# mrjoshuak/go-jpeg2000

Measured on AMD Instinct MI355X. Metric: Mpixels/s encode+decode (4K sRGB, 5-3 lossless), higher is better.
Workload: dtype int32

## Files before the change

### go-jpeg2000_amd/csrc/ht.hip

```cpp
#include <cstdlib>

#include "ht_tables.h"
#include "j2k_internal.h"

namespace j2k {

__device__ __constant__ uint16_t c_vlc_tbl0[1024] = J2K_HT_VLC_TBL0_INIT;
__device__ __constant__ uint16_t c_vlc_tbl1[1024] = J2K_HT_VLC_TBL1_INIT;
__device__ uint16_t g_vlc_enc[2 * 4 * 16];

__global__ void ht_build_enc_table() {
    const int t = threadIdx.x;
    if (t >= 128) return;
    const int initial = t >> 6, context = (t >> 4) & 3, rho = t & 15;
    const uint16_t *tbl = initial ? c_vlc_tbl0 : c_vlc_tbl1;
    uint16_t r = 0x0001;
    for (uint32_t cwd = 0; cwd < 128; cwd++) {
        const uint16_t e = tbl[(context << 7) | cwd];
        if (((e >> 4) & 0xF) == rho && (e & 0xF) > 0) { r = (uint16_t)((cwd << 4) | (e & 0xF)); break; }
    }
    g_vlc_enc[t] = r;
}

__device__ uint16_t g_vlc_pair1[16384];
// ... 1207 lines not shown
    const v4i_ v = {a, b, c, d};
    if (J2K_DECODED_NT) __builtin_nontemporal_store(v, reinterpret_cast<v4i_ *>(p));
    else *reinterpret_cast<v4i_ *>(p) = v;
}

#ifdef J2K_DEC_STAMP
static __device__ long long g_dbg_unstuff_dummy;
#define g_dbg_unstuff S.dbg_t
#endif
struct HtDecShared {
#ifdef J2K_DEC_STAMP
    long long dbg_t;
#endif
    uint32_t mbuf[HT_DEC_MWORDS];
    uint32_t pair[HT_WALK_MAX_PAIRS];
    uint32_t ffpos[HT_MAX_FF];
    uint32_t nff;
};

__device__ uint32_t ht_loaded_bits(const HtDecShared &S, uint32_t nff, long segLen, uint32_t j) {
    const long k = 4 * (long)j;
    const long kk = k < segLen ? k : segLen;
    uint32_t f = 0, last_ff = 0;
    for (uint32_t i = 0; i < nff; i++) {
        if ((long)S.ffpos[i] + 2 <= kk) f++;
        if ((long)S.ffpos[i] == segLen - 1) last_ff = 1;
    }
    uint32_t b = (uint32_t)(8 * kk) - f;
    if (k > segLen) b += (last_ff ? 7u : 8u) + 7u * (uint32_t)(k - segLen - 1);
    return b;
}

template <bool STRIDED>
__device__ bool ht_extract_fast(HtDecShared &S, const uint8_t *__restrict__ data, long len, long scup, int w, int h,
                                int32_t *__restrict__ out, int lane, bool bigu, const uint32_t (&mpos2)[2], uint32_t total_bits,
                                const uint32_t (&raw0)[4], int os_) {
    const size_t os64 = STRIDED ? (size_t)os_ : (size_t)64, osw = STRIDED ? (size_t)os_ : (size_t)w;
    const int quadCols = (w + 3) / 4, P = (quadCols + 1) / 2, R = (h + 3) / 4, N = R * P;
    const long lcup = len;
    {
        const long segLen0 = lcup - scup;
        const long cap0 = (long)HT_DEC_MWORDS * 4 - 16;
        const uint32_t zw = bigu ? (uint32_t)HT_DEC_MWORDS
                                 : min((uint32_t)HT_DEC_MWORDS, (uint32_t)(((segLen0 < cap0 ? segLen0 : cap0) * 8) >> 5) + 3u);
        for (uint32_t i = lane; i < zw; i += 64) S.mbuf[i] = 0;
    }
    if (lane == 0) S.nff = 0;
    wave_sync();
    constexpr int PF = 4;
    {
        const long segLen = lcup - scup;
        const long maxbytes = (long)HT_DEC_MWORDS * 4 - 16;
        const long nb = segLen < maxbytes ? segLen : maxbytes;
        const long d = (long)((uintptr_t)data & 3);
        const uint32_t *wsrc = reinterpret_cast<const uint32_t *>(data - d);
        const long ndw = (d + nb + 3) >> 2;
        uint32_t off = 0, carry = 0;
        for (long j0 = 0; j0 < ndw; j0 += 64 * PF) {
            uint32_t raw[PF];
#pragma unroll
            for (int c = 0; c < PF; c++) {
                const long j = j0 + 64 * c + lane;
                if (j0 == 0) raw[c] = raw0[c];
                else raw[c] = wsrc[j < ndw ? j : ndw - 1];
            }
#pragma unroll
            for (int c = 0; c < PF; c++) {
// ... 137 lines not shown
#pragma unroll
            for (int half = 0; half < 2; half++) {
                const int drow = half * 4 + (lane >> 4), q = lane & 15;
                const int src = drow * 8 + (q >> 1);
                int o[4];
#pragma unroll
                for (int i = 0; i < 4; i++) {
                    const int a = __shfl(vals[i], src), b = __shfl(vals[4 + i], src);
                    o[i] = (q & 1) ? b : a;
                }
                const int rg = 8 * t + drow;
#ifdef J2K_DEC_NO_CODED_STORES
                if (o[0] == 0x7fffffff)
#endif
                if (rg < R) st_decoded(out + (size_t)(4 * rg) * os64 + 4 * q, o[0], o[1], o[2], o[3]);
            }
        } else if (it < N) {
            const int xb = pi * 8;
            int32_t *orow = out + (size_t)(4 * r) * osw + xb;
            if (xb + 8 <= w && (((uintptr_t)orow) & 15) == 0) {
                st_decoded(orow, vals[0], vals[1], vals[2], vals[3]);
                st_decoded(orow + 4, vals[4], vals[5], vals[6], vals[7]);
            } else {
#pragma unroll
                for (int i = 0; i < 8; i++)
                    if (xb + i < w) orow[i] = vals[i];
            }
        }
    }
    return true;
}

template <bool STRIDED>
__global__ __launch_bounds__(256) __attribute__((amdgpu_waves_per_eu(7, 8))) void ht_decode_kernel(const BlockJob *__restrict__ jobs, int njobs,
                                                        const uint8_t *__restrict__ stream, const uint64_t *__restrict__ offs,
                                                        const uint32_t *__restrict__ lens, int32_t *__restrict__ decoded,
                                                        const uint32_t *__restrict__ pairs, int coded_rows_only_) {
    const int coded_rows_only = STRIDED ? 1 : coded_rows_only_;
    __shared__ HtDecShared S4[4];
    HtDecShared &S = S4[threadIdx.x >> 6];
    const int jid = blockIdx.x * 4 + (threadIdx.x >> 6);
    if (jid >= njobs) return;
    const int lane = threadIdx.x & 63;
#ifdef J2K_DEC_STAMP
    const long long d0 = wall_clock64();
#endif
    const BlockJob J = jobs[jid];
    const int w = J.w, h = J.h;
    const int os_ = STRIDED ? J.stride : w;
    int32_t *out = decoded + J.out_off;
    const size_t n = (size_t)w * h;
    const uint32_t *rec = pairs + (size_t)jid * HT_WALK_REC;
    const uint32_t r0 = rec[lane], r1 = rec[64 + lane];
    const uint64_t my_off = offs[jid];
    const uint32_t my_len = lens[jid], my_scup = rec[HT_WALK_MAX_PAIRS];
    const uint32_t tag = __shfl(r0, 0);
    const bool fast = (tag != HT_PAIR_ZERO) && (tag != HT_PAIR_SERIAL);
    auto zero_fill = [&](bool skip_coded) {
        if (coded_rows_only) {
            if (skip_coded) return;
            const uint32_t uw = (uint32_t)w, nrow = (uint32_t)(h + 3) >> 2;
            for (uint32_t i = lane; i < uw * nrow; i += 64) out[(size_t)(i / uw) * 4 * (STRIDED ? (uint32_t)os_ : uw) + i % uw] = 0;
            return;
        }
        if (w == 64 && (J.out_off & 3) == 0) {
            if (skip_coded && lane < 16) return;
            int32_t *q = out + 4 * (size_t)lane;
            for (int i = 0; i < h / 4; i++) st_decoded(q + 256 * (size_t)i, 0, 0, 0, 0);
            const int rem = h & 3;
            if (lane < 16 * rem) st_decoded(q + 256 * (size_t)(h / 4), 0, 0, 0, 0);
        } else if ((w & 3) == 0 && (J.out_off & 3) == 0) {
            const uint32_t wq = (uint32_t)w >> 2, nq = (uint32_t)(n >> 2);
            const uint32_t dy = 64u / wq, dx = 64u % wq;
            uint32_t y = (uint32_t)lane / wq, x = (uint32_t)lane % wq;
            for (uint32_t i = lane; i < nq; i += 64) {
                if (!skip_coded || (y & 3)) st_decoded(out + 4 * (size_t)i, 0, 0, 0, 0);
// ... 140 lines not shown
        const uint16_t *tbl = initial ? c_vlc_tbl0 : c_vlc_tbl1;
        for (int qx = 0; qx < quadCols; qx += 2) {
            uint32_t vlcVal = rev_fetch(vlc);
            const uint32_t qinf = tbl[vlcVal & 0x7F];
            const uint32_t rho = (qinf >> 4) & 0xF, uOff1 = (qinf >> 3) & 1;
            rev_advance(vlc, qinf & 0xF);
            vlcVal = rev_fetch(vlc);
            const uint32_t qinf2 = tbl[((rho >> 2) << 7) | (vlcVal & 0x7F)];
            const uint32_t rho2 = (qinf2 >> 4) & 0xF, uOff2 = (qinf2 >> 3) & 1;
            rev_advance(vlc, qinf2 & 0xF);
            uint32_t u[2] = {1, 1};
            const uint32_t mode = (uOff1 << 1) | uOff2;
            if (mode > 0) {
                vlcVal = rev_fetch(vlc);
                rev_advance(vlc, decode_uvlc(vlcVal, mode, u, initial));
            }
            for (int q = 0; q < 2; q++) {
                const uint32_t r = q ? rho2 : rho, emb = u[q];
                const int base = (qx + q) * 4;
                for (int i = 0; i < 4 && base + i < w; i++) {
                    if (!((r >> i) & 1)) continue;
                    const uint32_t magVal = fwd_fetch(ms);
                    const uint32_t mag = (magVal & (shl32(1, emb) - 1)) + shl32(1, emb - 1);
                    fwd_advance(ms, emb);
                    const uint32_t sign = fwd_fetch(ms) & 1;
                    fwd_advance(ms, 1);
                    out[(size_t)y * (STRIDED ? (size_t)os_ : (size_t)w) + base + i] = sign ? (int32_t)(0u - mag) : (int32_t)mag;
                }
            }
        }
    }
}

static bool g_tables_ready[16] = {false};

static hipError_t ht_tables_ready(hipStream_t s) {
    int dev = 0;
    hipError_t e = hipGetDevice(&dev);
    if (e != hipSuccess) return e;
    if (dev < 0 || dev >= 16) return hipErrorInvalidDevice;
    if (g_tables_ready[dev]) return hipSuccess;
    hipLaunchKernelGGL(ht_build_enc_table, dim3(1), dim3(128), 0, s);
    hipLaunchKernelGGL(ht_build_pair_table, dim3(64), dim3(256), 0, s);
    if ((e = hipGetLastError()) != hipSuccess) return e;
    if ((e = hipFuncSetAttribute(reinterpret_cast<const void *>(ht_walk_kernel), hipFuncAttributeMaxDynamicSharedMemorySize,
                                 (int)sizeof(HtWalkShared))) != hipSuccess) return e;
    if ((e = hipStreamSynchronize(s)) != hipSuccess) return e;
    g_tables_ready[dev] = true;
    return hipSuccess;
}

hipError_t launch_ht_encode(hipStream_t s, const BlockJob *jobs, int njobs, const int32_t *coef, uint8_t *slots,
                            uint32_t *lens, uint8_t *numbps, int *fault, uint32_t *maglens, const HtUJob *utab, int nunique,
                            const int *alias_ids, int waves) {
    if (njobs <= 0) return hipSuccess;
    hipError_t e;
    if ((e = ht_tables_ready(s)) != hipSuccess) return e;
    const int n = utab ? nunique : njobs;
    if (waves == 4 && utab && alias_ids)
        hipLaunchKernelGGL(ht_encode_wg_kernel, dim3(n), dim3(256), 0, s, n, coef, slots, lens, numbps, fault, maglens, utab, alias_ids);
    else
        hipLaunchKernelGGL(ht_encode_kernel, dim3(n), dim3(64), 0, s, jobs, n, coef, slots, lens, numbps, fault, maglens, utab, alias_ids);
    return hipGetLastError();
}

hipError_t launch_ht_encode_stream(hipStream_t s, const BlockJob *jobs, int njobs, const int32_t *coef, uint8_t *stream,
                                   uint64_t *offs, uint32_t *lens, uint8_t *numbps, uint64_t *status, uint32_t epoch, int *fault) {
    if (njobs <= 0) return hipSuccess;
    hipError_t e;
    if ((e = ht_tables_ready(s)) != hipSuccess) return e;
    hipLaunchKernelGGL(ht_encode_stream_kernel, dim3(njobs), dim3(64), 0, s, jobs, njobs, coef, stream,
                       reinterpret_cast<unsigned long long *>(offs), lens, numbps, reinterpret_cast<unsigned long long *>(status), epoch, fault);
    return hipGetLastError();
}
int ht_fast_max_samples() { return HT_FAST_MAX_SAMPLES; }

size_t ht_decode_scratch_words(int njobs) { return (size_t)njobs * (HT_WALK_REC + HT_VBITS_WORDS); }

hipError_t launch_ht_decode(hipStream_t s, const BlockJob *jobs, int njobs, const uint8_t *stream, const uint64_t *offs,
                            const uint32_t *lens, int32_t *decoded, uint32_t *scratch, int coded_rows_only, const BlockJob *placed_jobs) {
    if (njobs <= 0) return hipSuccess;
    hipError_t e;
    if ((e = ht_tables_ready(s)) != hipSuccess) return e;
    uint32_t *pairs = scratch, *vbits = scratch + (size_t)njobs * HT_WALK_REC;
    for (int rep_ = 0; rep_ < dev_reps(32); rep_++)
    hipLaunchKernelGGL(ht_vlcprep_kernel, dim3((njobs + 3) / 4), dim3(256), 0, s, jobs, njobs, stream, offs, lens, vbits, pairs);
    if ((e = hipGetLastError()) != hipSuccess) return e;
    for (int rep_ = 0; rep_ < dev_reps(64); rep_++)
    hipLaunchKernelGGL(ht_walk_kernel, dim3((njobs + HT_WALK_BLOCKS - 1) / HT_WALK_BLOCKS), dim3(256), sizeof(HtWalkShared), s, jobs, njobs, vbits, pairs);
    if ((e = hipGetLastError()) != hipSuccess) return e;
    for (int rep_ = 0; rep_ < dev_reps(128); rep_++)
    if (placed_jobs) hipLaunchKernelGGL(ht_decode_kernel<true>, dim3((njobs + 3) / 4), dim3(256), 0, s, placed_jobs, njobs, stream, offs, lens, decoded, pairs, 1);
    else
    hipLaunchKernelGGL(ht_decode_kernel<false>, dim3((njobs + 3) / 4), dim3(256), 0, s, jobs, njobs, stream, offs, lens, decoded, pairs, coded_rows_only);
    return hipGetLastError();
}

}
```

### go-jpeg2000_amd/csrc/j2k_ctx.cpp

```cpp
#include "j2k_host.h"

using namespace j2k;

int fail(j2k_ctx *ctx, int status, const char *msg) {
    if (ctx) ctx->last_error = msg ? msg : "";
    return status;
}
int fail_hip(j2k_ctx *ctx, hipError_t e, const char *where) {
    char buf[256];
    snprintf(buf, sizeof(buf), "%s: %s", where, hipGetErrorString(e));
    if (ctx) ctx->last_error = buf;
    return J2K_ERR_HIP;
}

extern "C" const char *j2k_ctx_last_error(j2k_ctx *ctx) { return ctx ? ctx->last_error.c_str() : ""; }

std::atomic<int> g_mq_ctxs{0};
bool mq_throughput_mode() { return g_mq_ctxs.load(std::memory_order_relaxed) >= 2; }
struct CtxOption { const char *name; bool (*set)(j2k_ctx *, long); };
static const std::vector<CtxOption> &ctx_options() {
#define OPT(name, cond, stmt) CtxOption{name, [](j2k_ctx *c, long v) -> bool { (void)c; if (!(cond)) return false; stmt; return true; }}
    static const std::vector<CtxOption> T = {
        OPT("plane_wg3", v == 0 || v == 1, c->plane_wg3 = v != 0),
        OPT("pix_fuse", v >= 0 && v <= 2, c->pix_fuse = (int)v),
        OPT("plane_wg", v == 0 || v == 4 || v == 8, c->plane_wg = (int)v),
        OPT("l0_fuse", v == 0 || v == 8 || v == 10 || v == 16, c->l0_fuse = (int)v),
        OPT("l0_wg", v == 0 || v == 4 || v == 8, c->l0_wg = (int)v),
        OPT("plane_wg97", v == 0 || v == 8, c->plane_wg97 = (int)v),
        OPT("l0_wg97_inv", v == 0 || v == 6 || v == 8 || v == 10 || v == 12, c->l0_wg97_inv = (int)v),
        OPT("l0_wg97", v == 0 || (v >= 6 && v <= 16 && v % 2 == 0), c->l0_wg97 = (int)v),
        OPT("l0_xcd", v == 0 || v == 1, c->l0_xcd = v != 0),
        OPT("l0_deal", v == 0 || v == 1, c->l0_deal = v != 0),
        OPT("ht_alias", v == 0 || v == 1, c->ht_alias = v != 0),
        OPT("ht_enc_waves", v == 1 || v == 4, c->ht_enc_waves = (int)v),
        OPT("l0_inv_wpe", v >= 5 && v <= 7, c->l0_inv_wpe = (int)v),
        OPT("l0_wg_inv", v == 0 || v == 1, c->l0_wg_inv = v != 0),
        OPT("l0_wg_invw", v == 0 || v == 4 || v == 8, c->l0_wg_invw = (int)v),
        OPT("l0_xcd_group", v >= 0 && v <= 4096, c->l0_xcd_group = (int)v),
        OPT("l0_store", v == 0 || v == 1 || v == 2 || v == 4, c->l0_store = (int)v),
        OPT("fuse_compact", v == 0 || v == 1, c->fuse_compact = v != 0),
        OPT("deep", v == 0 || v == 1, c->use_deep = v != 0),
        OPT("deep_min_planes", v >= 0 && v <= 1000000, c->deep_min_planes = (int)v),
        OPT("deep_mid", v == 0 || v == 1, c->deep_mid = v != 0),
        OPT("deep_mid_inv", v >= 0 && v <= 2, c->deep_mid_inv = (int)v),
        OPT("mega", v >= 0 && v <= 2, c->mega = (int)v),
        OPT("t1_split", v == 0 || v == 1, c->t1_split = v != 0),
        OPT("t1_sym_mb", v >= 0, c->t1_sym_mb = v),
        OPT("t1_dec_general", v == 0 || v == 1, c->t1_dec_general = v != 0),
        OPT("t1_dec_split", v >= -1, c->t1_dec_split = (int)v),
        OPT("t1_dec_lanes", v >= 0 && v <= 2, c->t1_dec_lanes = (int)v),
        OPT("t1_lanes", v >= 0 && v <= 64, c->t1_lanes = (int)v),
        OPT("t2_parallel", v == 0 || v == 1, c->t2_parallel = v != 0),
    };
#undef OPT
    return T;
}
extern "C" int j2k_ctx_set_option(j2k_ctx *ctx, const char *name, long value) {
    if (!ctx || !name) return J2K_ERR_INVALID_ARG;
    for (const CtxOption &o : ctx_options())
        if (!strcmp(o.name, name)) return o.set(ctx, value) ? J2K_OK : fail(ctx, J2K_ERR_INVALID_ARG, "j2k_ctx_set_option: value out of range");
    return fail(ctx, J2K_ERR_INVALID_ARG, "j2k_ctx_set_option: no such option");
}

extern "C" int j2k_ctx_create(int device, j2k_ctx **out) {
    if (!out) return J2K_ERR_INVALID_ARG;
    *out = nullptr;
    int n = 0;
// ... 173 lines not shown
```

### go-jpeg2000_amd/csrc/j2k_frame.cpp

```cpp
#include "j2k_host.h"

using namespace j2k;

extern "C" int j2k_t2_encode_packets_device(j2k_ctx *ctx, const j2k_t2_dev_packet *d_packets, size_t npackets, const j2k_t2_dev_cb *d_cbs, size_t ncbs,
                                            const uint8_t *d_data, int sop, int eph, uint8_t *bio_delay, uint8_t *d_out, size_t cap,
                                            uint64_t *d_offs, size_t *total) {
    if (!ctx || !bio_delay || !d_offs || !total || (npackets && !d_packets) || (ncbs && !d_cbs) || (cap && !d_out)) return J2K_ERR_INVALID_ARG;
    if (ctx->capturing) return fail(ctx, J2K_ERR_INVALID_ARG, "a synchronising call while the context captures a graph");
    if (npackets > ((size_t)1 << 31)) return fail(ctx, J2K_ERR_INVALID_ARG, "too many packets");
    HIPCHK(ctx, hipSetDevice(ctx->device));
    const size_t ws = j2k::t2_dev_workspace((long)npackets);
    int r = stage_reserve(ctx, 1, ws + 64);
    if (r != J2K_OK) return r;
    uint64_t *d_res = reinterpret_cast<uint64_t *>((uint8_t *)ctx->stage[1] + ((ws + 15) & ~size_t(15)));
    HIPCHK(ctx, hipMemsetAsync(d_res, 0, 3 * sizeof(uint64_t), ctx->stream));
    HIPCHK(ctx, j2k::launch_t2_encode_packets(ctx->stream, d_packets, (long)npackets, d_cbs, (uint64_t)ncbs, d_data, sop, eph, *bio_delay ? 1 : 0, d_out, (uint64_t)cap,
                                              d_offs, ctx->stage[1], d_res));
    uint64_t res[3] = {0, 0, 0};
    HIPCHK(ctx, hipMemcpyAsync(res, d_res, sizeof(res), hipMemcpyDeviceToHost, ctx->stream));
    HIPCHK(ctx, hipStreamSynchronize(ctx->stream));
    if (res[2]) return fail(ctx, J2K_ERR_GO_PANIC, "packet coder: a tag tree of width 0 (the reference divides by it, t2.go:328,348), or a packet whose code-blocks lie outside the table");
    *total = (size_t)res[0];
    if (res[0] > cap) return fail(ctx, J2K_ERR_CAPACITY, "packet coder: the output buffer is smaller than the packets");
    *bio_delay = res[1] ? 1 : 0;
// ... 249 lines not shown
    return r;
}

extern "C" int j2k_plan_encode_frame_image(j2k_plan *P, const j2k_image *d_img, int sop, int eph, uint8_t *d_out, size_t cap, uint64_t *d_tile_offs) {
    if (!P || !d_img) return J2K_ERR_INVALID_ARG;
    if (!d_out || !d_tile_offs) return fail(P->ctx, J2K_ERR_INVALID_ARG, "null device pointer");
    int r = cl_prepare(P);
    if (r == J2K_OK) r = cl_workspaces(P);
    if (r == J2K_OK) r = plan_forward_image_impl(P, d_img, P->d_cl_coeff, P->d_frame_status);
    if (r == J2K_OK) r = plan_encode_frame_from_coeff(P, P->d_cl_coeff, P->d_cl_lens, P->d_cl_numbps, sop, eph, d_out, cap, d_tile_offs);
    return r;
}

static int decode_frame_pixels_impl(j2k_plan *P, const uint8_t *d_cs, size_t len, const uint64_t *d_tile_offs, int sop, int eph, int skip_planes, void *d_pix,
                                    size_t stride);
static int decode_frame_pixels_reduced_impl(j2k_plan *P, const uint8_t *d_cs, size_t len, const uint64_t *d_tile_offs, int sop, int eph, int reduce,
                                            int skip_planes, void *d_pix, size_t stride);
extern "C" int j2k_plan_decode_frame_pixels(j2k_plan *P, const uint8_t *d_cs, size_t len, const uint64_t *d_tile_offs, int sop, int eph, void *d_pix,
                                            size_t stride) {
    return decode_frame_pixels_impl(P, d_cs, len, d_tile_offs, sop, eph, 0, d_pix, stride);
}
static int decode_frame_pixels_impl(j2k_plan *P, const uint8_t *d_cs, size_t len, const uint64_t *d_tile_offs, int sop, int eph, int skip_planes, void *d_pix,
                                    size_t stride) {
    if (!P) return J2K_ERR_INVALID_ARG;
    int r = cl_prepare(P);
    if (r == J2K_OK) r = cl_workspaces(P);
    if (r == J2K_OK) r = j2k_plan_decode_tile_parts(P, d_cs, len, d_tile_offs, sop, eph, P->d_cl_offs, P->d_cl_lens, P->d_cl_numbps);
    if (r != J2K_OK) return r;
    if (P->spec.coder == J2K_CODER_HT) {
        j2k_ctx *ctx = P->ctx;
        const int n = (int)P->blocks.size();
        r = stage_reserve(ctx, 2, ht_decode_scratch_words(n) * 4 + 256);
        if (r != J2K_OK) return r;
        HIPCHK(ctx, launch_ht_decode(ctx->stream, P->d_djobs, n, d_cs, P->d_cl_offs, P->d_cl_lens, P->d_cl_coeff_dec, (uint32_t *)ctx->stage[2], 1, P->d_djobs_placed));
        return plan_inverse_pixels_impl(P, P->d_cl_coeff_dec, d_pix, stride, P->d_frame_status);
    } else {
        r = j2k_plan_decode_blocks_coarse(P, d_cs, P->d_cl_offs, P->d_cl_lens, P->d_cl_numbps, skip_planes, P->d_cl_decoded);
        if (r == J2K_OK) r = j2k_plan_place_blocks(P, P->d_cl_decoded, P->d_cl_coeff);
    }
    if (r == J2K_OK) r = plan_inverse_pixels_impl(P, P->d_cl_coeff, d_pix, stride, P->d_frame_status);
    return r;
}

extern "C" int j2k_plan_decode_frame_pixels_reduced(j2k_plan *P, const uint8_t *d_cs, size_t len, const uint64_t *d_tile_offs, int sop, int eph, int reduce,
                                                    void *d_pix, size_t stride) {
    return decode_frame_pixels_reduced_impl(P, d_cs, len, d_tile_offs, sop, eph, reduce, 0, d_pix, stride);
}
static int decode_frame_pixels_reduced_impl(j2k_plan *P, const uint8_t *d_cs, size_t len, const uint64_t *d_tile_offs, int sop, int eph, int reduce,
                                            int skip_planes, void *d_pix, size_t stride) {
    if (!P) return J2K_ERR_INVALID_ARG;
    j2k_ctx *ctx = P->ctx;
    ReducedTab *R = nullptr;
    int r = plan_reduced(P, reduce, &R);
    if (r != J2K_OK) return r;
    if (reduce == 0) return decode_frame_pixels_impl(P, d_cs, len, d_tile_offs, sop, eph, skip_planes, d_pix, stride);
    if (!d_pix) return fail(ctx, J2K_ERR_INVALID_ARG, "null device pointer");
    r = cl_prepare(P);
    if (r == J2K_OK) r = cl_workspaces(P);
    if (r == J2K_OK) r = j2k_plan_decode_tile_parts(P, d_cs, len, d_tile_offs, sop, eph, P->d_cl_offs, P->d_cl_lens, P->d_cl_numbps);
    if (r != J2K_OK) return r;
    HIPCHK(ctx, launch_select_blocks(ctx->stream, R->d_ids, R->njobs, P->d_cl_offs, P->d_cl_lens, P->d_cl_numbps, R->d_offs, R->d_lens, R->d_numbps));
    const bool ht = P->spec.coder == J2K_CODER_HT;
    int32_t *coeff = ht ? P->d_cl_coeff_dec : P->d_cl_coeff;
    r = plan_decode_blocks_jobs(P, R->d_djobs, R->njobs, d_cs, R->d_offs, R->d_lens, R->d_numbps, ht ? coeff : P->d_cl_decoded, ht ? R->d_placed : nullptr, skip_planes);
    if (r == J2K_OK && !ht) HIPCHK(ctx, launch_place_blocks(ctx->stream, R->d_bjobs, R->d_djobs, R->njobs, R->max_block_h, P->d_cl_decoded, coeff));
    if (r == J2K_OK) r = plan_inverse_pixels_reduced_impl(P, coeff, reduce, d_pix, stride, P->d_frame_status);
    return r;
// ... 106 lines not shown
```

### go-jpeg2000_amd/csrc/j2k_host.h

```cpp
#pragma once
#include <algorithm>
#include <atomic>
#include <cstdio>
#include <cstdlib>
#include <cstring>
#include <map>
#include <tuple>

#include "j2k_plan.h"

namespace j2k {
#ifdef J2K_DEV
int g_dev_skip = 0, g_dev_dup = 0;
#endif
hipError_t launch_add_const(hipStream_t s, int32_t *d, size_t n, int delta);
hipError_t launch_rct(hipStream_t s, int32_t *a, int32_t *b, int32_t *c, size_t n, int inverse);
hipError_t launch_ict(hipStream_t s, double *a, double *b, double *c, size_t n, int inverse);
hipError_t launch_dwt97_fwd(hipStream_t s, const LevelLaunch &L, const void *src, int src_is_f64, int32_t *out_i32,
                            double *out_f64, double *nxt, int dc_shift, int quant, double step, int mct);
hipError_t launch_dwt97_inv(hipStream_t s, const LevelLaunch &L, const void *coef, int coef_is_f64, const double *prev,
                            void *dst, int dc_shift, int final_level, int dst_mode, int mct, double step);
hipError_t launch_quantize97(hipStream_t s, const double *src, size_t n, double step, int32_t *dst);
hipError_t launch_dequantize97(hipStream_t s, const int32_t *src, size_t n, double step, double *dst);
hipError_t launch_ht_encode(hipStream_t s, const BlockJob *jobs, int njobs, const int32_t *coef, uint8_t *slots,
                            uint32_t *lens, uint8_t *numbps, int *fault, uint32_t *maglens = nullptr, const HtUJob *utab = nullptr, int nunique = 0,
                            const int *alias_ids = nullptr, int waves = 1);
hipError_t launch_ht_decode(hipStream_t s, const BlockJob *jobs, int njobs, const uint8_t *stream, const uint64_t *offs,
                            const uint32_t *lens, int32_t *decoded, uint32_t *scratch, int coded_rows_only = 0, const BlockJob *placed_jobs = nullptr);
size_t ht_decode_scratch_words(int njobs);
hipError_t launch_ht_encode_stream(hipStream_t s, const BlockJob *jobs, int njobs, const int32_t *coef, uint8_t *stream,
                                   uint64_t *offs, uint32_t *lens, uint8_t *numbps, uint64_t *status, uint32_t epoch, int *fault);
int ht_fast_max_samples();
hipError_t launch_t1_encode(hipStream_t s, const BlockJob *jobs, int njobs, const int32_t *coef, uint8_t *slots,
                            uint32_t *lens, uint8_t *numbps, uint8_t *work, size_t work_per_job, int *fault, int max_dim,
                            uint8_t *sym, size_t sym_stride, uint32_t *nsyms, int lanes, uint8_t *bigsym = nullptr, const uint64_t *bigsym_off = nullptr,
                            uint32_t *bignsyms = nullptr, uint32_t *rate = nullptr);
hipError_t launch_rate_distortion(hipStream_t s, const BlockJob *jobs, int njobs, const int32_t *coef, const uint8_t *numbps, uint64_t *dist);
size_t rate_allocate_workspace(int njobs);
hipError_t launch_rate_allocate(hipStream_t s, int njobs, const uint32_t *rate, const uint64_t *dist, const uint8_t *numbps, const double *weights,
                                uint64_t budget, void *ws, uint8_t *kept, uint64_t *chosen);
hipError_t launch_rate_allocate_layers(hipStream_t s, int njobs, const uint32_t *rate, const uint64_t *dist, const uint8_t *numbps, const double *weights,
                                       const uint64_t *budgets, int nlayers, void *ws, uint8_t *kept, uint64_t *chosen);
hipError_t launch_t2_fill_layer_cbs(hipStream_t s, long n, int nlayers, const uint64_t *offs, const BlockJob *slot_jobs, const uint32_t *lens, const uint8_t *numbps,
                                    int mb, const uint8_t *kept, const uint32_t *rate, j2k_t2_dev_cb *cbs, uint64_t *reset);
hipError_t launch_t2_layer_ends(hipStream_t s, int count, int nlayers, const int *end_packet, const uint64_t *poffs, uint64_t *layer_offs);
hipError_t launch_t2_decode_tiles_layers(hipStream_t s, void *chains, int ntiles, const j2k_t2_dev_packet *packets, long npackets, j2k_t2_dev_cb *cbs, long n,
                                         int nlayers, const uint8_t *data, uint64_t len, int sop, int eph, uint64_t *body_base, int *frame_status, int mb,
                                         uint8_t *dense, uint64_t dense_cap, uint64_t *offs, uint32_t *lens, uint8_t *numbps, uint8_t *floors);
size_t t1_sym_stride(int planes);
hipError_t launch_t1_decode(hipStream_t s, const BlockJob *jobs, int njobs, const uint8_t *stream, const uint64_t *offs,
                            const uint32_t *lens, const uint8_t *numbps, int32_t *decoded, uint8_t *work,
                            size_t work_per_job, int max_dim, int general_only, uint8_t *split_ws, int sig_lanes, int throughput = 0, int skip_planes = 0,
                            const uint8_t *floors = nullptr);
size_t t1_dec_split_bytes(size_t njobs);
hipError_t launch_mq_encode(hipStream_t s, const uint8_t *ctxs, const uint8_t *decs, size_t n, uint8_t *out, size_t cap, uint32_t *out_len, int *fault);
hipError_t launch_mq_decode(hipStream_t s, const uint8_t *data, size_t len, const uint8_t *ctxs, size_t n, uint8_t *decs, int *fault);
hipError_t launch_raw_encode(hipStream_t s, const uint8_t *bits, size_t n, uint8_t *out, size_t cap, uint32_t *out_len, int *fault);
hipError_t launch_raw_decode(hipStream_t s, const uint8_t *data, size_t len, size_t n, uint8_t *bits);
size_t t1_work_bytes(int w, int h);
size_t t1_flag_bytes(int w, int h);
hipError_t launch_compact(hipStream_t s, const BlockJob *jobs, int njobs, const uint8_t *slots, const uint32_t *lens,
// ... 89 lines not shown
```

### go-jpeg2000_amd/csrc/j2k_hostcalls.cpp

```cpp
#include "j2k_host.h"

using namespace j2k;

int cached_plan(j2k_ctx *ctx, const PlanSpec &S, j2k_plan **out) {
    for (j2k_plan *p : ctx->cache)
        if (p->spec == S) { *out = p; return J2K_OK; }
    j2k_plan *p = nullptr;
    int r = build_plan(ctx, S, &p);
    if (r != J2K_OK) return r;
    if (ctx->cache.size() >= 16) { j2k_plan_destroy(ctx->cache.front()); ctx->cache.erase(ctx->cache.begin()); }
    ctx->cache.push_back(p);
    *out = p;
    return J2K_OK;
}

static int host_dwt(j2k_ctx *ctx, void *data, int w, int h, int levels, int wavelet, bool inverse, int quant, bool frame_f64) {
    if (!ctx) return J2K_ERR_INVALID_ARG;
    if (w < 0 || h < 0 || levels < 0) return fail(ctx, J2K_ERR_INVALID_ARG, "negative size");
    if (w == 0 || h == 0 || levels == 0) return J2K_OK;
    if (!data) return fail(ctx, J2K_ERR_INVALID_ARG, "data == NULL");
    HIPCHK(ctx, hipSetDevice(ctx->device));
    PlanSpec S;
    S.W = w; S.H = h; S.C = 1; S.levels = levels; S.wavelet = wavelet; S.dc_shift = 0; S.dc_shift_inv = 0; S.mct = 0;
    S.quant = quant; S.frame_is_f64 = frame_f64; S.num_res_jobs = 1; S.cb_w = 1 << 20; S.cb_h = 1 << 20;
// ... 217 lines not shown
    HIPCHK(ctx, hipSetDevice(ctx->device));
    size_t nbytes = 0;
    std::vector<BlockJob> bj(nblocks);
    int64_t dec = 0;
    size_t wpj = 0;
    for (size_t j = 0; j < nblocks; j++) {
        const j2k_block &b = blocks[j];
        if (b.w <= 0 || b.h <= 0 || b.band < 0 || b.band > 3) return fail(ctx, J2K_ERR_INVALID_ARG, "bad block");
        nbytes = std::max<size_t>(nbytes, (size_t)offs[j] + lens[j]);
        bj[j].src_off = 0; bj[j].out_off = dec; bj[j].stride = b.w; bj[j].w = b.w; bj[j].h = b.h; bj[j].band = b.band;
        dec += align4((int64_t)b.w * b.h);
        wpj = std::max(wpj, t1_flag_bytes(b.w, b.h));
    }
    if (nbytes && !bytes) return fail(ctx, J2K_ERR_INVALID_ARG, "bytes == NULL");
    wpj = (wpj + 255) & ~size_t(255);
    void *d_bytes = nullptr, *d_jobs = nullptr, *d_offs = nullptr, *d_lens = nullptr, *d_nb = nullptr, *d_dec = nullptr, *d_work = nullptr, *d_floors = nullptr;
    int status = J2K_OK;
    auto cleanup = [&]() { for (void *p : {d_bytes, d_jobs, d_offs, d_lens, d_nb, d_dec, d_work, d_floors}) if (p) (void)hipFree(p); };
    TRY(hipMalloc(&d_bytes, nbytes + 16));
    if (floors) { TRY(hipMalloc(&d_floors, nblocks + 16)); TRY(hipMemcpyAsync(d_floors, floors, nblocks, hipMemcpyHostToDevice, ctx->stream)); }
    TRY(hipMalloc(&d_jobs, nblocks * sizeof(BlockJob)));
    TRY(hipMalloc(&d_offs, nblocks * 8));
    TRY(hipMalloc(&d_lens, nblocks * 4));
    TRY(hipMalloc(&d_nb, nblocks));
    TRY(hipMalloc(&d_dec, (size_t)dec * 4 + 16));
    if (nbytes) TRY(hipMemcpyAsync(d_bytes, bytes, nbytes, hipMemcpyHostToDevice, ctx->stream));
    TRY(hipMemcpyAsync(d_jobs, bj.data(), nblocks * sizeof(BlockJob), hipMemcpyHostToDevice, ctx->stream));
    TRY(hipMemcpyAsync(d_offs, offs, nblocks * 8, hipMemcpyHostToDevice, ctx->stream));
    TRY(hipMemcpyAsync(d_lens, lens, nblocks * 4, hipMemcpyHostToDevice, ctx->stream));
    if (numbps) TRY(hipMemcpyAsync(d_nb, numbps, nblocks, hipMemcpyHostToDevice, ctx->stream));
    else TRY(hipMemsetAsync(d_nb, 0, nblocks, ctx->stream));
    if (coder == J2K_CODER_HT) {
        TRY(hipMalloc(&d_work, ht_decode_scratch_words((int)nblocks) * 4 + 256));
        TRY(launch_ht_decode(ctx->stream, (BlockJob *)d_jobs, (int)nblocks, (uint8_t *)d_bytes, (uint64_t *)d_offs, (uint32_t *)d_lens, (int32_t *)d_dec, (uint32_t *)d_work));
    } else {
        const int split_min = ctx->t1_dec_split >= 0 ? ctx->t1_dec_split : (mq_throughput_mode() ? 512 : 12000);
        bool split = split_min > 0 && (int)nblocks >= split_min && !ctx->t1_dec_general;
        const size_t gen_bytes = (wpj * nblocks + 255) & ~size_t(255);
        if (split && hipMalloc(&d_work, gen_bytes + 256 + j2k::t1_dec_split_bytes(nblocks)) != hipSuccess) { (void)hipGetLastError(); d_work = nullptr; split = false; }
        if (!split) TRY(hipMalloc(&d_work, gen_bytes + 256));
        int max_dim = 0;
        for (size_t j = 0; j < nblocks; j++) max_dim = std::max(max_dim, std::max(bj[j].w, bj[j].h));
        TRY(launch_t1_decode(ctx->stream, (BlockJob *)d_jobs, (int)nblocks, (uint8_t *)d_bytes, (uint64_t *)d_offs, (uint32_t *)d_lens, (uint8_t *)d_nb,
                             (int32_t *)d_dec, (uint8_t *)d_work, wpj, max_dim, ctx->t1_dec_general, split ? (uint8_t *)d_work + gen_bytes : nullptr, ctx->t1_dec_lanes, 0, skip_planes, (const uint8_t *)d_floors));
    }
    for (size_t j = 0; j < nblocks; j++)
        TRY(hipMemcpyAsync(coeffs + coeff_offs[j], (int32_t *)d_dec + bj[j].out_off, (size_t)blocks[j].w * blocks[j].h * 4, hipMemcpyDeviceToHost, ctx->stream));
    TRY(hipStreamSynchronize(ctx->stream));
    cleanup();
    return J2K_OK;
}
#undef TRY

extern "C" int j2k_encode_frame(j2k_plan *P, int32_t *const *planes, int32_t *coeff, uint8_t *out, size_t cap,
                                size_t *out_len, uint64_t *tile_offs, uint32_t *lens, uint8_t *numbps) {
    if (!P || !planes) return J2K_ERR_INVALID_ARG;
    j2k_ctx *ctx = P->ctx;
    const PlanSpec &S = P->spec;
    HIPCHK(ctx, hipSetDevice(ctx->device));
    const size_t npx = (size_t)S.W * S.H;
    const size_t nb = P->blocks.size();
    int r;
    if ((r = ensure(ctx, &P->d_frame, npx * S.C * 4)) != J2K_OK) return r;
    if ((r = ensure(ctx, &P->d_coeff, (size_t)P->coeff_elems * 4)) != J2K_OK) return r;
    if ((r = ensure(ctx, &P->d_slots, (size_t)P->bytes_cap)) != J2K_OK) return r;
    if ((r = ensure(ctx, &P->d_stream, (size_t)P->bytes_cap)) != J2K_OK) return r;
    if ((r = ensure(ctx, &P->d_lens, nb * 4)) != J2K_OK) return r;
// ... 213 lines not shown
```

### go-jpeg2000_amd/csrc/j2k_plan.h

```cpp
#pragma once
#include <string>
#include <vector>

#include "../../include/j2kgfx.h"
#include "j2k_internal.h"

struct j2k_ctx {
    int device = -1;
    hipStream_t stream = nullptr;
    std::string last_error;
    int fuse_compact = 0;
    int fwd_link = 1;
    int inv_link = 1;
    int pix_fuse = 1;
    bool plane_wg3 = false;
    int plane_wg = 4;
    int l0_fuse = 0;
    int l0_wg = 8;
    int l0_wg_invw = 4;
    bool l0_deal = true;
    int l0_wg97 = 8;
    int plane_wg97 = 8;
    int l0_wg97_inv = 8;
    int l0_xcd_group = 16;
    bool l0_xcd = true;
    bool ht_alias = true;
    int ht_enc_waves = 4;
    int l0_inv_wpe = 5;
    bool l0_wg_inv = true;
    int l0_store = 1;
    int band_prows_pix = 3;
    int band_prows_97 = 8;
    int band_prows_inv = 0;
    int fwd_pf = 0;
    int band_prows = 5;
    int use_tail = 1;
    int mega = 0;
    int deep_mid_inv = 1;
    int deep_min_planes = 12;
    int deep_mid = 1;
    int use_deep = 1;
    int xcd_map = 0;
    int cpl0 = 0;
    int force_novec = 0;
    int t1_split = 1;
    long t1_sym_mb = 8192;
    int t1_dec_general = 0;
    int t1_dec_lanes = 2;
    int t1_dec_split = -1;
    bool capturing = false;
    bool fault_armed_before_capture = false;
    bool counted_mq = false;
    bool t2_parallel = true;
    int t1_lanes = 0;
    std::vector<j2k_plan *> cache;
    void *stage[5] = {nullptr, nullptr, nullptr, nullptr, nullptr};
    bool fault_armed = false;
    size_t stage_bytes[5] = {0, 0, 0, 0, 0};
    int profile = 0;
    std::vector<hipEvent_t> ev;
// ... 178 lines not shown
```

### go-jpeg2000_amd/csrc/j2k_stages.cpp

```cpp
#include "j2k_host.h"

using namespace j2k;

static LevelLaunch mk(const LevelTab &T, int pf = 0) {
    LevelLaunch L{T.d_jobs, T.njobs, T.d_planes, T.cpl, T.vec, T.ncomp, pf};
    L.pjobs = T.d_pjobs; L.pnjobs = T.p_pix_only ? 0 : T.pnjobs; L.pwaves = T.pwaves; L.pmulti = T.pmulti;
    L.mallat = T.mallat ? 1 : 0;
    return L;
}

static void pix_launch(LevelLaunch &L, const LevelTab &T, const PixIO &pix, int cls, const PlanSpec &S) {
    L.pix_stride = pix.stride;
    L.pix_src = cls ? (pix.triple == 4 ? 4 : 0) : pix.single;
    L.comp_elems = (long long)S.W * S.H;
    if (cls == 1 && pix.triple == 4) L.pnjobs = T.pnjobs;
}

int plan_forward_impl(j2k_plan *P, const void *d_frame, void *d_coeff, PixIO pix) {
    const int pix_stride = pix.stride;
    j2k_ctx *ctx = P->ctx;
    const PlanSpec &S = P->spec;
    if (((uintptr_t)d_frame & 15) || ((uintptr_t)d_coeff & 15)) return fail(ctx, J2K_ERR_INVALID_ARG, "device pointers must be 16-byte aligned");
    HIPCHK(ctx, hipSetDevice(ctx->device));
    const double step = 1.0 / (double)S.quality;
// ... 785 lines not shown
int check_skip_planes(j2k_ctx *ctx, int coder, int skip_planes, const char *who) {
    if (skip_planes < 0 || skip_planes > 31) return fail(ctx, J2K_ERR_INVALID_ARG, (std::string(who) + ": skip_planes outside 0 ... 31").c_str());
    if (skip_planes > 0 && coder == J2K_CODER_HT)
        return fail(ctx, J2K_ERR_UNSUPPORTED, (std::string(who) + ": skip_planes > 0 needs the MQ coder (the HT coder's one pass has no planes to stop between)").c_str());
    return J2K_OK;
}

extern "C" int j2k_plan_decode_blocks_coarse(j2k_plan *P, const uint8_t *d_stream, const uint64_t *d_offs, const uint32_t *d_lens,
                                             const uint8_t *d_numbps, int skip_planes, int32_t *d_decoded) {
    if (!P || !d_stream || !d_offs || !d_lens || !d_numbps || !d_decoded) return J2K_ERR_INVALID_ARG;
    const int r = check_skip_planes(P->ctx, P->spec.coder, skip_planes, "j2k_plan_decode_blocks_coarse");
    if (r != J2K_OK) return r;
    return plan_decode_blocks_jobs(P, P->d_djobs, (int)P->blocks.size(), d_stream, d_offs, d_lens, d_numbps, d_decoded, nullptr, skip_planes);
}

extern "C" int j2k_plan_decode_blocks_floors(j2k_plan *P, const uint8_t *d_stream, const uint64_t *d_offs, const uint32_t *d_lens,
                                             const uint8_t *d_numbps, int skip_planes, const uint8_t *d_floors, int32_t *d_decoded) {
    if (!P || !d_stream || !d_offs || !d_lens || !d_numbps || !d_decoded) return J2K_ERR_INVALID_ARG;
    const int r = check_skip_planes(P->ctx, P->spec.coder, skip_planes, "j2k_plan_decode_blocks_floors");
    if (r != J2K_OK) return r;
    if (d_floors && P->spec.coder == J2K_CODER_HT) return fail(P->ctx, J2K_ERR_UNSUPPORTED, "j2k_plan_decode_blocks_floors: per-block floors need the MQ coder");
    return plan_decode_blocks_jobs(P, P->d_djobs, (int)P->blocks.size(), d_stream, d_offs, d_lens, d_numbps, d_decoded, nullptr, skip_planes, d_floors);
}

int plan_decode_blocks_jobs(j2k_plan *P, const BlockJob *d_djobs, int n, const uint8_t *d_stream, const uint64_t *d_offs, const uint32_t *d_lens,
                            const uint8_t *d_numbps, int32_t *d_decoded, const BlockJob *d_placed, int skip_planes, const uint8_t *d_floors) {
    j2k_ctx *ctx = P->ctx;
    HIPCHK(ctx, hipSetDevice(ctx->device));
    if (!n) return J2K_OK;
    if (P->spec.coder == J2K_CODER_HT) {
        int r = stage_reserve(ctx, 2, ht_decode_scratch_words(n) * 4 + 256);
        if (r != J2K_OK) return r;
        HIPCHK(ctx, launch_ht_decode(ctx->stream, d_djobs, n, d_stream, d_offs, d_lens, d_decoded, (uint32_t *)ctx->stage[2],
                                     (d_placed || P->dec_coded_rows_only) ? 1 : 0, d_placed));
    } else {
        size_t wpj = 0;
        int max_dim = 0;
        for (const j2k_block &b : P->blocks) { wpj = std::max(wpj, t1_flag_bytes(b.w, b.h)); max_dim = std::max(max_dim, std::max(b.w, b.h)); }
        wpj = (wpj + 255) & ~size_t(255);
        const int split_min = ctx->t1_dec_split >= 0 ? ctx->t1_dec_split : (mq_throughput_mode() ? 512 : 12000);
        bool split = split_min > 0 && n >= split_min && !ctx->t1_dec_general && !((uintptr_t)d_stream & 15);
        const size_t gen_bytes = (wpj * (size_t)n + 255) & ~size_t(255);
        int r = stage_reserve(ctx, 2, gen_bytes + 256 + (split ? j2k::t1_dec_split_bytes((size_t)n) : 0));
        if (r != J2K_OK && split) { (void)hipGetLastError(); split = false; r = stage_reserve(ctx, 2, gen_bytes + 256); }
        if (r != J2K_OK) return r;
        HIPCHK(ctx, launch_t1_decode(ctx->stream, d_djobs, n, d_stream, d_offs, d_lens, d_numbps, d_decoded,
                                     (uint8_t *)ctx->stage[2], wpj, max_dim, ctx->t1_dec_general,
                                     split ? (uint8_t *)ctx->stage[2] + gen_bytes : nullptr, ctx->t1_dec_lanes, mq_throughput_mode() ? 1 : 0, skip_planes, d_floors));
    }
    return J2K_OK;
}
```

Measured before the change: 79590.

## Add lean HT decode kernel specialized for power-of-two block widths

```diff
diff --git a/go-jpeg2000_amd/csrc/ht.hip b/go-jpeg2000_amd/csrc/ht.hip
--- a/go-jpeg2000_amd/csrc/ht.hip
+++ b/go-jpeg2000_amd/csrc/ht.hip
@@ -1263,7 +1263,7 @@
 }
 
 template <bool STRIDED>
-__device__ bool ht_extract_fast(HtDecShared &S, const uint8_t *__restrict__ data, long len, long scup, int w, int h,
+__device__ __forceinline__ bool ht_extract_fast(HtDecShared &S, const uint8_t *__restrict__ data, long len, long scup, int w, int h,
                                 int32_t *__restrict__ out, int lane, bool bigu, const uint32_t (&mpos2)[2], uint32_t total_bits,
                                 const uint32_t (&raw0)[4], int os_) {
     const size_t os64 = STRIDED ? (size_t)os_ : (size_t)64, osw = STRIDED ? (size_t)os_ : (size_t)w;
@@ -1467,16 +1467,11 @@
 }
 
 template <bool STRIDED>
-__global__ __launch_bounds__(256) __attribute__((amdgpu_waves_per_eu(7, 8))) void ht_decode_kernel(const BlockJob *__restrict__ jobs, int njobs,
-                                                        const uint8_t *__restrict__ stream, const uint64_t *__restrict__ offs,
-                                                        const uint32_t *__restrict__ lens, int32_t *__restrict__ decoded,
-                                                        const uint32_t *__restrict__ pairs, int coded_rows_only_) {
+__device__ __forceinline__ void ht_decode_block(HtDecShared &S, const int jid, const int lane, const BlockJob *__restrict__ jobs,
+                                                const uint8_t *__restrict__ stream, const uint64_t *__restrict__ offs,
+                                                const uint32_t *__restrict__ lens, int32_t *__restrict__ decoded,
+                                                const uint32_t *__restrict__ pairs, int coded_rows_only_) {
     const int coded_rows_only = STRIDED ? 1 : coded_rows_only_;
-    __shared__ HtDecShared S4[4];
-    HtDecShared &S = S4[threadIdx.x >> 6];
-    const int jid = blockIdx.x * 4 + (threadIdx.x >> 6);
-    if (jid >= njobs) return;
-    const int lane = threadIdx.x & 63;
 #ifdef J2K_DEC_STAMP
     const long long d0 = wall_clock64();
 #endif
@@ -1683,6 +1678,199 @@
     }
 }
 
+template <bool STRIDED>
+__global__ __launch_bounds__(256) __attribute__((amdgpu_waves_per_eu(7, 8))) void ht_decode_kernel(const BlockJob *__restrict__ jobs, int njobs,
+                                                        const uint8_t *__restrict__ stream, const uint64_t *__restrict__ offs,
+                                                        const uint32_t *__restrict__ lens, int32_t *__restrict__ decoded,
+                                                        const uint32_t *__restrict__ pairs, int coded_rows_only_) {
+    __shared__ HtDecShared S4[4];
+    const int jid = blockIdx.x * 4 + (threadIdx.x >> 6);
+    if (jid >= njobs) return;
+    ht_decode_block<STRIDED>(S4[threadIdx.x >> 6], jid, threadIdx.x & 63, jobs, stream, offs, lens, decoded, pairs, coded_rows_only_);
+}
+
+template <bool STRIDED>
+__global__ __launch_bounds__(256) __attribute__((amdgpu_waves_per_eu(7, 8))) void ht_decode_lean_kernel(const BlockJob *__restrict__ jobs, int njobs,
+                                                        const uint8_t *__restrict__ stream, const uint64_t *__restrict__ offs,
+                                                        const uint32_t *__restrict__ lens, int32_t *__restrict__ decoded,
+                                                        const uint32_t *__restrict__ pairs, int coded_rows_only_) {
+    const int coded_rows_only = STRIDED ? 1 : coded_rows_only_;
+    __shared__ HtDecShared S4[4];
+    const int wave = __builtin_amdgcn_readfirstlane((int)(threadIdx.x >> 6));
+    HtDecShared &S = S4[wave];
+    const int jid = blockIdx.x * 4 + wave;
+    if (jid >= njobs) return;
+    const int lane = threadIdx.x & 63;
+    const BlockJob J = jobs[jid];
+    const int w = J.w, h = J.h;
+    const uint32_t os = STRIDED ? (uint32_t)J.stride : (uint32_t)w;
+    int32_t *out = decoded + J.out_off;
+    const uint32_t *rec = pairs + (size_t)jid * HT_WALK_REC;
+    const uint32_t rr[2] = {rec[lane], rec[64 + lane]};
+    const uint64_t my_off = offs[jid];
+    const uint32_t my_len = lens[jid], my_scup = rec[HT_WALK_MAX_PAIRS];
+    const uint32_t tag = (uint32_t)__builtin_amdgcn_readfirstlane((int)rr[0]);
+    const bool lean = tag != HT_PAIR_ZERO && tag != HT_PAIR_SERIAL && (w == 64 || w == 32 || w == 16 || w == 8) && (((uintptr_t)out) & 15) == 0 &&
+                      (!STRIDED || (os & 3) == 0);
+    if (lean) {
+    const uint32_t psh = (uint32_t)__builtin_ctz((unsigned)w) - 3, P = 1u << psh;
+    const uint32_t R = (uint32_t)(h + 3) >> 2, N = R << psh;
+    const uint8_t *data = stream + my_off;
+    const long segLen = (long)my_len - (long)my_scup;
+    const long maxbytes = (long)HT_DEC_MWORDS * 4 - 16;
+    const uint32_t nb = (uint32_t)(segLen < maxbytes ? segLen : maxbytes);
+    const uint32_t d = (uint32_t)((uintptr_t)data & 3);
+    const uint32_t *wsrc = reinterpret_cast<const uint32_t *>(data - d);
+    const uint32_t ndw = (d + nb + 3) >> 2;
+    uint32_t raw0[4] = {0, 0, 0, 0};
+    if (ndw > 0) {
+#pragma unroll
+        for (int c = 0; c < 4; c++) {
+            const uint32_t j = 64 * c + lane;
+            raw0[c] = wsrc[j < ndw ? j : ndw - 1];
+        }
+    }
+    if (!coded_rows_only) {
+        const uint32_t nq = (uint32_t)(w * h) >> 2, qsh = psh + 1;
+        for (uint32_t i = lane; i < nq; i += 64)
+            if ((i >> qsh) & 3) st_decoded(out + 4 * i, 0, 0, 0, 0);
+    }
+    uint32_t info2[2] = {0, 0}, mpos2[2] = {0, 0}, total_bits = 0;
+    bool bigu = false;
+#pragma unroll
+    for (int t = 0; t < 2; t++) {
+        if (64u * t >= N) break;
+        const uint32_t it = lane + 64 * t;
+        const uint32_t r = rr[t], mode = (r >> 13) & 3, vw = r >> 16;
+        const uint32_t t1 = (mode & 1) ? uvlc_entry(vw) : 0u;
+        const uint32_t pl1 = t1 & 3;
+        const uint32_t v1 = vw >> pl1;
+        const uint32_t t2 = (mode & 2) ? uvlc_entry(v1) : 0u;
+        const uint32_t pl2 = t2 & 3;
+        const uint32_t v2 = v1 >> pl2;
+        const uint32_t sl1 = (t1 >> 2) & 7, sl2 = (t2 >> 2) & 7;
+        uint32_t a = (t1 >> 5) + (v2 & ((1u << sl1) - 1)) + 1;
+        uint32_t b = (t2 >> 5) + ((v2 >> sl1) & ((1u << sl2) - 1)) + 1;
+        if (t == 0) {
+            const bool first = it < P && mode == 3 && pl1 == 3;
+            a = first ? (t1 >> 5) + ((v1 >> 1) & ((1u << sl1) - 1)) + 1 : a;
+            b = first ? (v1 & 1) + 2 : b;
+        }
+        const bool live = it < N;
+        if (live && (a > 31 || b > 31)) bigu = true;
+        const uint32_t rhos = live ? (r & 0xFF) : 0u;
+        info2[t] = rhos | a << 8 | b << 14;
+        const uint32_t nbits = __popc(rhos & 0xF) * (a + 1) + __popc(rhos >> 4) * (b + 1);
+        const uint32_t ns = wave_incl_scan(nbits);
+        mpos2[t] = total_bits + ns - nbits;
+        total_bits += wave_last(ns);
+    }
+    if (!__any(bigu)) {
+    {
+        const uint32_t zw = min((uint32_t)HT_DEC_MWORDS, ((nb * 8) >> 5) + 3u);
+        for (uint32_t i = lane; i < zw; i += 64) S.mbuf[i] = 0;
+    }
+    wave_sync();
+    constexpr int PF = 4;
+    uint32_t off = 0, carry = 0;
+    for (uint32_t j0 = 0; j0 < ndw; j0 += 64 * PF) {
+        uint32_t raw[PF];
+#pragma unroll
+        for (int c = 0; c < PF; c++) {
+            const uint32_t j = j0 + 64 * c + lane;
+            if (j0 == 0) raw[c] = raw0[c];
+            else raw[c] = wsrc[j < ndw ? j : ndw - 1];
+        }
+#pragma unroll
+        for (int c = 0; c < PF; c++) {
+            if (j0 + 64 * c >= ndw) break;
+            const uint32_t j = j0 + 64 * c + lane;
+            const uint32_t dw = raw[c];
+            uint32_t prev3 = __shfl_up(dw >> 24, 1);
+            if (lane == 0) prev3 = carry;
+            carry = __shfl(dw >> 24, 63);
+            const int k0 = (int)(4 * j) - (int)d;
+            uint32_t wd[4], tot = 0;
+            bool plain = (j < ndw) && k0 >= 1 && k0 + 4 <= (int)nb && prev3 != 0xFF;
+#pragma unroll
+            for (int t = 0; t < 4; t++) {
+                const int k = k0 + t;
+                const uint32_t pb = t ? ((dw >> (8 * (t - 1))) & 0xFF) : prev3;
+                const bool valid = (j < ndw) && k >= 0 && k < (int)nb;
+                wd[t] = valid ? ((k > 0 && pb == 0xFF) ? 7u : 8u) : 0u;
+                if (t && pb == 0xFF) plain = false;
+                tot += wd[t];
+            }
+            const uint32_t ws = wave_incl_scan(tot);
+            uint32_t pos = off + ws - tot;
+            if (plain) {
+                if (dw) or_bits(S.mbuf, pos, (uint64_t)dw);
+            } else {
+#pragma unroll
+                for (int t = 0; t < 4; t++) {
+                    const uint32_t bt = (dw >> (8 * t)) & 0xFF;
+                    if (wd[t] && bt) or_bits(S.mbuf, pos, (uint64_t)bt);
+                    pos += wd[t];
+                }
+            }
+            off += wave_last(ws);
+        }
+    }
+    wave_sync();
+    if ((long)nb == segLen) {
+        const uint32_t wd0 = off >> 5;
+        const uint32_t wend = min((uint32_t)HT_DEC_MWORDS, (total_bits >> 5) + 3u);
+        for (uint32_t i = wd0 + lane; i < wend; i += 64)
+            S.mbuf[i] = (i == wd0) ? (S.mbuf[i] | (0xFFFFFFFFu << (off & 31))) : 0xFFFFFFFFu;
+    }
+    wave_sync();
+#pragma unroll
+    for (int t = 0; t < 2; t++) {
+        if (64u * t >= N) break;
+        uint32_t mpos = mpos2[t];
+        int vals[8];
+        const uint32_t info = info2[t], u0 = (info >> 8) & 0x3F, u1 = (info >> 14) & 0x3F;
+        const uint32_t half0 = 1u << (u0 - 1), half1 = 1u << (u1 - 1);
+#pragma unroll
+        for (int i = 0; i < 8; i++) {
+            const uint32_t emb = (i < 4) ? u0 : u1;
+            const bool on = (info >> i) & 1;
+            const uint32_t wd = mpos >> 5;
+            const uint32_t win = __builtin_amdgcn_alignbit(S.mbuf[wd + 1], S.mbuf[wd], mpos & 31);
+            const uint32_t mag = __builtin_amdgcn_ubfe(win, 0, emb) + ((i < 4) ? half0 : half1);
+            const uint32_t sg = 0u - ((win >> emb) & 1);
+            vals[i] = on ? (int32_t)((mag ^ sg) - sg) : 0;
+            mpos += on ? emb + 1 : 0u;
+        }
+        if (w != 64) {
+            const uint32_t it = lane + 64 * t;
+            int32_t *orow = out + (4 * (it >> psh) * os + 8 * (it & (P - 1)));
+            if (it < N) {
+                st_decoded(orow, vals[0], vals[1], vals[2], vals[3]);
+                st_decoded(orow + 4, vals[4], vals[5], vals[6], vals[7]);
+            }
+            continue;
+        }
+#pragma unroll
+        for (int half = 0; half < 2; half++) {
+            const uint32_t drow = half * 4 + (lane >> 4), q = lane & 15;
+            const int src = (int)(drow * 8 + (q >> 1));
+            int o[4];
+#pragma unroll
+            for (int i = 0; i < 4; i++) {
+                const int a = __shfl(vals[i], src), b = __shfl(vals[4 + i], src);
+                o[i] = (q & 1) ? b : a;
+            }
+            const uint32_t rg = 8 * t + drow;
+            if (rg < R) st_decoded(out + (4 * rg * os + 4 * q), o[0], o[1], o[2], o[3]);
+        }
+    }
+    return;
+    }
+    }
+    ht_decode_block<STRIDED>(S, jid, lane, jobs, stream, offs, lens, decoded, pairs, coded_rows_only_);
+}
+
 static bool g_tables_ready[16] = {false};
 
 static hipError_t ht_tables_ready(hipStream_t s) {
@@ -1729,7 +1917,7 @@
 size_t ht_decode_scratch_words(int njobs) { return (size_t)njobs * (HT_WALK_REC + HT_VBITS_WORDS); }
 
 hipError_t launch_ht_decode(hipStream_t s, const BlockJob *jobs, int njobs, const uint8_t *stream, const uint64_t *offs,
-                            const uint32_t *lens, int32_t *decoded, uint32_t *scratch, int coded_rows_only, const BlockJob *placed_jobs) {
+                            const uint32_t *lens, int32_t *decoded, uint32_t *scratch, int coded_rows_only, const BlockJob *placed_jobs, int lean) {
     if (njobs <= 0) return hipSuccess;
     hipError_t e;
     if ((e = ht_tables_ready(s)) != hipSuccess) return e;
@@ -1741,9 +1929,9 @@
     hipLaunchKernelGGL(ht_walk_kernel, dim3((njobs + HT_WALK_BLOCKS - 1) / HT_WALK_BLOCKS), dim3(256), sizeof(HtWalkShared), s, jobs, njobs, vbits, pairs);
     if ((e = hipGetLastError()) != hipSuccess) return e;
     for (int rep_ = 0; rep_ < dev_reps(128); rep_++)
-    if (placed_jobs) hipLaunchKernelGGL(ht_decode_kernel<true>, dim3((njobs + 3) / 4), dim3(256), 0, s, placed_jobs, njobs, stream, offs, lens, decoded, pairs, 1);
+    if (placed_jobs) hipLaunchKernelGGL(lean ? ht_decode_lean_kernel<true> : ht_decode_kernel<true>, dim3((njobs + 3) / 4), dim3(256), 0, s, placed_jobs, njobs, stream, offs, lens, decoded, pairs, 1);
     else
-    hipLaunchKernelGGL(ht_decode_kernel<false>, dim3((njobs + 3) / 4), dim3(256), 0, s, jobs, njobs, stream, offs, lens, decoded, pairs, coded_rows_only);
+    hipLaunchKernelGGL(lean ? ht_decode_lean_kernel<false> : ht_decode_kernel<false>, dim3((njobs + 3) / 4), dim3(256), 0, s, jobs, njobs, stream, offs, lens, decoded, pairs, coded_rows_only);
     return hipGetLastError();
 }
 
diff --git a/go-jpeg2000_amd/csrc/j2k_ctx.cpp b/go-jpeg2000_amd/csrc/j2k_ctx.cpp
--- a/go-jpeg2000_amd/csrc/j2k_ctx.cpp
+++ b/go-jpeg2000_amd/csrc/j2k_ctx.cpp
@@ -33,6 +33,7 @@
         OPT("l0_deal", v == 0 || v == 1, c->l0_deal = v != 0),
         OPT("ht_alias", v == 0 || v == 1, c->ht_alias = v != 0),
         OPT("ht_enc_waves", v == 1 || v == 4, c->ht_enc_waves = (int)v),
+        OPT("ht_dec_lean", v == 0 || v == 1, c->ht_dec_lean = (int)v),
         OPT("l0_inv_wpe", v >= 5 && v <= 7, c->l0_inv_wpe = (int)v),
         OPT("l0_wg_inv", v == 0 || v == 1, c->l0_wg_inv = v != 0),
         OPT("l0_wg_invw", v == 0 || v == 4 || v == 8, c->l0_wg_invw = (int)v),
diff --git a/go-jpeg2000_amd/csrc/j2k_frame.cpp b/go-jpeg2000_amd/csrc/j2k_frame.cpp
--- a/go-jpeg2000_amd/csrc/j2k_frame.cpp
+++ b/go-jpeg2000_amd/csrc/j2k_frame.cpp
@@ -305,7 +305,7 @@
         const int n = (int)P->blocks.size();
         r = stage_reserve(ctx, 2, ht_decode_scratch_words(n) * 4 + 256);
         if (r != J2K_OK) return r;
-        HIPCHK(ctx, launch_ht_decode(ctx->stream, P->d_djobs, n, d_cs, P->d_cl_offs, P->d_cl_lens, P->d_cl_coeff_dec, (uint32_t *)ctx->stage[2], 1, P->d_djobs_placed));
+        HIPCHK(ctx, launch_ht_decode(ctx->stream, P->d_djobs, n, d_cs, P->d_cl_offs, P->d_cl_lens, P->d_cl_coeff_dec, (uint32_t *)ctx->stage[2], 1, P->d_djobs_placed, ctx->ht_dec_lean));
         return plan_inverse_pixels_impl(P, P->d_cl_coeff_dec, d_pix, stride, P->d_frame_status);
     } else {
         r = j2k_plan_decode_blocks_coarse(P, d_cs, P->d_cl_offs, P->d_cl_lens, P->d_cl_numbps, skip_planes, P->d_cl_decoded);
diff --git a/go-jpeg2000_amd/csrc/j2k_host.h b/go-jpeg2000_amd/csrc/j2k_host.h
--- a/go-jpeg2000_amd/csrc/j2k_host.h
+++ b/go-jpeg2000_amd/csrc/j2k_host.h
@@ -26,7 +26,7 @@
                             uint32_t *lens, uint8_t *numbps, int *fault, uint32_t *maglens = nullptr, const HtUJob *utab = nullptr, int nunique = 0,
                             const int *alias_ids = nullptr, int waves = 1);
 hipError_t launch_ht_decode(hipStream_t s, const BlockJob *jobs, int njobs, const uint8_t *stream, const uint64_t *offs,
-                            const uint32_t *lens, int32_t *decoded, uint32_t *scratch, int coded_rows_only = 0, const BlockJob *placed_jobs = nullptr);
+                            const uint32_t *lens, int32_t *decoded, uint32_t *scratch, int coded_rows_only = 0, const BlockJob *placed_jobs = nullptr, int lean = 1);
 size_t ht_decode_scratch_words(int njobs);
 hipError_t launch_ht_encode_stream(hipStream_t s, const BlockJob *jobs, int njobs, const int32_t *coef, uint8_t *stream,
                                    uint64_t *offs, uint32_t *lens, uint8_t *numbps, uint64_t *status, uint32_t epoch, int *fault);
diff --git a/go-jpeg2000_amd/csrc/j2k_hostcalls.cpp b/go-jpeg2000_amd/csrc/j2k_hostcalls.cpp
--- a/go-jpeg2000_amd/csrc/j2k_hostcalls.cpp
+++ b/go-jpeg2000_amd/csrc/j2k_hostcalls.cpp
@@ -273,7 +273,7 @@
     else TRY(hipMemsetAsync(d_nb, 0, nblocks, ctx->stream));
     if (coder == J2K_CODER_HT) {
         TRY(hipMalloc(&d_work, ht_decode_scratch_words((int)nblocks) * 4 + 256));
-        TRY(launch_ht_decode(ctx->stream, (BlockJob *)d_jobs, (int)nblocks, (uint8_t *)d_bytes, (uint64_t *)d_offs, (uint32_t *)d_lens, (int32_t *)d_dec, (uint32_t *)d_work));
+        TRY(launch_ht_decode(ctx->stream, (BlockJob *)d_jobs, (int)nblocks, (uint8_t *)d_bytes, (uint64_t *)d_offs, (uint32_t *)d_lens, (int32_t *)d_dec, (uint32_t *)d_work, 0, nullptr, ctx->ht_dec_lean));
     } else {
         const int split_min = ctx->t1_dec_split >= 0 ? ctx->t1_dec_split : (mq_throughput_mode() ? 512 : 12000);
         bool split = split_min > 0 && (int)nblocks >= split_min && !ctx->t1_dec_general;
diff --git a/go-jpeg2000_amd/csrc/j2k_plan.h b/go-jpeg2000_amd/csrc/j2k_plan.h
--- a/go-jpeg2000_amd/csrc/j2k_plan.h
+++ b/go-jpeg2000_amd/csrc/j2k_plan.h
@@ -26,6 +26,7 @@
     bool l0_xcd = true;
     bool ht_alias = true;
     int ht_enc_waves = 4;
+    int ht_dec_lean = 1;
     int l0_inv_wpe = 5;
     bool l0_wg_inv = true;
     int l0_store = 1;
diff --git a/go-jpeg2000_amd/csrc/j2k_stages.cpp b/go-jpeg2000_amd/csrc/j2k_stages.cpp
--- a/go-jpeg2000_amd/csrc/j2k_stages.cpp
+++ b/go-jpeg2000_amd/csrc/j2k_stages.cpp
@@ -841,7 +841,7 @@
         int r = stage_reserve(ctx, 2, ht_decode_scratch_words(n) * 4 + 256);
         if (r != J2K_OK) return r;
         HIPCHK(ctx, launch_ht_decode(ctx->stream, d_djobs, n, d_stream, d_offs, d_lens, d_decoded, (uint32_t *)ctx->stage[2],
-                                     (d_placed || P->dec_coded_rows_only) ? 1 : 0, d_placed));
+                                     (d_placed || P->dec_coded_rows_only) ? 1 : 0, d_placed, ctx->ht_dec_lean));
     } else {
         size_t wpj = 0;
         int max_dim = 0;
```

New measurement: 81220, median of 6. +2.1%, better.
